# SnappyDataInc/snappydata

Hardware: AMD Instinct MI355X
Metric: rows/sec scan+filter+agg (TPC-H lineitem) (higher is better)
Workload: dtype f64; 1 GPU; tpch_q6_lineitem_sf100; rows_per_gpu=600000000, total_rows=600000000, bytes_per_row=28, batch_rows=600000, parallelism=bucket-dp1, jit=True

## Files before the change

### include/snappy_engine.h

```cpp
#ifndef SNAPPY_ENGINE_H
#define SNAPPY_ENGINE_H

#include <stdint.h>
#include <stddef.h>

#ifdef __cplusplus
extern "C" {
#endif

#define SN_OK                0
#define SN_ERR_GENERIC      -1
#define SN_ERR_BADARG       -2
#define SN_ERR_NOMEM        -3
#define SN_ERR_BADFORMAT    -4
#define SN_ERR_UNSUPPORTED  -5
#define SN_ERR_NOGPU        -6
#define SN_ERR_OVERFLOW     -7

typedef enum {
  SN_TYPE_INT32  = 0,
  SN_TYPE_INT64  = 1,
  SN_TYPE_DOUBLE = 2,
  SN_TYPE_STRING = 3,
  SN_TYPE_BOOL   = 4,
// ... 135 lines not shown
                           double *dict, int32_t *ndict);

int32_t sn_dim_define(sn_engine *e, const char *name);
int32_t sn_dim_put(sn_engine *e, int32_t dim, int64_t nkeys,
                   const int64_t *keys, const char *attr_payload,
                   const int32_t *attr_lens);

int32_t sn_dim_from_table(sn_engine *e, int32_t dim, int32_t table,
                          int32_t key_col, int32_t attr_col);

int32_t sn_batch_mutate(sn_engine *e, int32_t table, int64_t uuid,
                        int32_t bucket_id, const sn_buf *delete_mask,
                        const sn_buf *deltas, const sn_buf *stats);

sn_query *sn_query_submit(sn_engine *e, const sn_plan *plan);
int32_t   sn_query_wait(sn_query *q);
int32_t   sn_query_result(sn_query *q, sn_result *out);
void      sn_query_destroy(sn_query *q);
double    sn_query_kernel_ms(sn_query *q);
int32_t   sn_query_result_page(sn_query *q, int64_t offset, sn_result *out);
int64_t   sn_query_num_groups(sn_query *q);
int32_t   sn_query_used_jit(sn_query *q);
int64_t   sn_query_late_cols(sn_query *q);
int32_t   sn_query_order_by(sn_query *q, int32_t agg_idx, int32_t descending,
                            int64_t k);

int64_t sn_query_partial_bytes(sn_query *q);
int32_t sn_query_partials(sn_query *q, void *dst, int32_t dst_is_device);
int64_t sn_query_partial_bytes2(sn_query *q, int32_t cap_slots);
int32_t sn_query_partials2(sn_query *q, void *dst, int32_t dst_is_device,
                           int32_t cap_slots);
int32_t sn_query_partials_sharded2(sn_query *q, int32_t world, void *dst,
                                   int32_t cap_slots);
int32_t sn_query_partials_sharded(sn_query *q, int32_t world, void *dst);
int32_t sn_query_merge(sn_query *q, const void *blocks, int64_t stride,
                       int32_t n_blocks);

typedef struct {
  int32_t col, _pad;
  int64_t add, mul;
} sn_dec_factor;

typedef struct {
  int32_t kind, nfactors;
  sn_dec_factor factors[SN_MAX_FACTORS];
} sn_dec_agg;
// ... 57 lines not shown
```

### snappydata_amd/csrc/engine.cpp

```cpp
#include <hip/hip_runtime.h>
#include <dlfcn.h>

#include <algorithm>
#include <atomic>
#include <climits>
#include <cmath>
#include <cstdarg>
#include <cstdio>
#include <cstring>
#include <malloc.h>
#include <limits>
#include <map>
#include <set>
#include <memory>
#include <mutex>
#include <string>
#include <thread>
#include <vector>

#include "../../include/snappy_engine.h"
#include "engine_internal.h"
#include "blob_format.h"
#include "partial_format.h"

// ... 148 lines not shown
  std::vector<int64_t> keys;
  std::vector<std::string> attrs;
  std::vector<std::string> attr_dict;
  std::vector<int32_t> attr_gid;
  const int64_t *dev_keys = nullptr;
  const int32_t *dev_payload = nullptr;
  int32_t cap_log2 = 0;
  const int32_t *dev_lut = nullptr;
  int64_t lut_min = 0, lut_max = -1;
  int32_t attr_maxlen = 0;
  bool from_table = false;
  std::mutex mu;
};

struct sn_engine {
  sn_config cfg;
  Arena arena;
  std::vector<std::unique_ptr<Table>> tables;
  std::vector<std::unique_ptr<Dim>> dims;
  hipStream_t stream = nullptr;
  bool has_gpu = false;
  bool narrow = true;
  bool late = true, late_force = false;
  double *scratch = nullptr;
  size_t scratch_sz = 0;
  long long *hws_keys = nullptr;
  long long *hws_okeys = nullptr;
  double *hws_acc = nullptr;
  double *hws_orows = nullptr;
  int32_t *hws_flags = nullptr;
  int hws_cap_log2 = 0;
  size_t hws_acc_bytes = 0;
  double *rws_recs = nullptr;
  size_t rws_bytes = 0;
  int32_t *rws_pcount = nullptr;
  int rws_npart = 0;
  int32_t *lz4_err_dev = nullptr;
  std::mutex lz4_mu;
  std::mutex query_mu;
  static const int PIN_SLOTS = 4;
  struct PinSlot { void *buf = nullptr; size_t sz = 0; std::mutex mu; };
  PinSlot pins[PIN_SLOTS];
  std::atomic<uint32_t> pin_rr { 0 };
  void *jit = nullptr;
  std::map<uint64_t, void *> dp_cache;
  std::vector<hipEvent_t> ev_pool;
// ... 10 lines not shown
  }
  void ev_release(hipEvent_t ev) {
    if (!ev) return;
    std::lock_guard<std::mutex> g(aux_mu);
    if (ev_pool.size() < 16) ev_pool.push_back(ev);
    else (void)hipEventDestroy(ev);
  }
};

extern "C" sn_engine *sn_engine_create(const sn_config *cfg) {
  auto *e = new sn_engine();
  if (cfg) e->cfg = *cfg;
  else memset(&e->cfg, 0, sizeof(e->cfg));
  if (e->cfg.column_batch_size <= 0) e->cfg.column_batch_size = 24ll << 20;
  if (e->cfg.column_max_delta_rows <= 0) e->cfg.column_max_delta_rows = 10000;
  if (e->cfg.hash_join_size <= 0) e->cfg.hash_join_size = 100ll << 20;
  if (e->cfg.shard_count <= 0) e->cfg.shard_count = 1;
  if (e->cfg.n_buckets <= 0) e->cfg.n_buckets = 128;
  if (const char *nv = getenv("SN_NARROW")) e->narrow = nv[0] != '0';
  if (const char *lv = getenv("SN_LATE")) {
    e->late = lv[0] != '0';
    e->late_force = !strcmp(lv, "force");
  }
  int ndev = 0;
  if (hipGetDeviceCount(&ndev) == hipSuccess && ndev > 0 && e->cfg.device >= 0) {
    if (hipSetDevice(e->cfg.device) == hipSuccess &&
        hipStreamCreate(&e->stream) == hipSuccess) {
      e->has_gpu = true;
      e->arena.device = e->cfg.device;
    }
  }
  if (!e->has_gpu) {
    e->arena.device = -1;
  } else {
    e->jit = sn_jit_cache_create();
  }
  (void)mallopt(M_MMAP_THRESHOLD, 256 << 20);
  (void)mallopt(M_TRIM_THRESHOLD, 256 << 20);
  return e;
}

static hipError_t d2h_copy(sn_engine *e, void *dst, const void *src, size_t n) {
  if (n < (1u << 20))
    return hipMemcpy(dst, src, n, hipMemcpyDeviceToHost);
  auto &slot = e->pins[e->pin_rr.fetch_add(1) % sn_engine::PIN_SLOTS];
  std::lock_guard<std::mutex> g(slot.mu);
// ... 1173 lines not shown
  bool mm = false;
  std::unique_ptr<long long[]> sparse_keys;
  std::unique_ptr<double[]> sparse_rows;
  size_t sparse_n = 0;
  std::vector<double> sparse_null_row;
  bool gint[2] = { false, false };
  int64_t gmin[2] = { 0, 0 };
  int gnull1 = -1, gnull2 = -1;
  int agg_map[SN_MAX_AGGS];
  int dev_naggs = 0;
  Dim *join_dim = nullptr;
  bool join_group = false;
  double *dev_out = nullptr;
  size_t out_stride = 0;
  int na_t = 0;
  std::vector<double> host_out;
  int64_t rows_scanned = 0;
  int64_t batches_seen = 0, batches_skipped = 0;
  hipEvent_t ev_start = nullptr, ev_stop = nullptr;
  std::vector<std::pair<void *, size_t>> owned;
  float kernel_ms = -1.0f;
  bool used_jit = false;
  int64_t late_cols = 0;
  bool done = false;
  bool merged = false;
  std::vector<GroupOut> final_groups;
  bool dec = false;
  int dec_ndev = 0;
  int dec_map[SN_MAX_AGGS];
  int dec_scale_of[SN_MAX_AGGS];
  unsigned long long *dec_out = nullptr;
  std::vector<sn_dec_val> dec_vals;
  bool select = false;
  int sel_nproj = 0;
  int32_t sel_cols[SN_SEL_MAX_PROJ];
  int64_t sel_limit = 0;
  int64_t sel_total = 0;
  int64_t sel_rows = 0;
  int sel_width[SN_SEL_MAX_PROJ];
  void *sel_val[SN_SEL_MAX_PROJ];
  uint8_t *sel_valid[SN_SEL_MAX_PROJ];
  int sel_kernels = 0;
  bool ordered = false;
  int32_t ord_col = 0, ord_flags = 0;
  int32_t rjoin = -1;
  float sel_ms[3] = { 0.0f, 0.0f, 0.0f };
// ... 927 lines not shown
}

static uint32_t tag_late_columns(const sn_query *q, const sn_dev_plan &dp,
                                 int *kinds) {
  const sn_engine *e = q->e;
  const sn_plan *plan = &q->plan;
  if (!e->late || plan->ngroup > 0 || q->join_dim || q->sparse || dp.nslots > 1)
    return 0;
  uint32_t agg = 0, other = 0;
  for (int a = 0; a < dp.naggs; a++) {
    const sn_dev_agg &A = dp.aggs[a];
    if (A.nf >= 1) agg |= 1u << A.c0;
    if (A.nf >= 2) agg |= 1u << A.c1;
    if (A.nf >= 3) agg |= 1u << A.c2;
  }
  for (int i = 0; i < dp.npreds_d; i++) other |= 1u << dp.preds_d[i].cslot;
  for (int i = 0; i < dp.npreds_i; i++) other |= 1u << dp.preds_i[i].cslot;
  for (int i = 0; i < dp.npreds_in && i < 2; i++) other |= 1u << dp.inp[i].cslot;
  uint32_t mask = 0;
  for (int ui = 0; ui < dp.nused; ui++)
    if (kinds[ui] == SN_K_F64 && ((agg & ~other) >> ui & 1)) mask |= 1u << ui;
  if (!mask || !other) return 0;
  if (!e->late_force && !(estimate_selectivity(q) <= SN_LATE_MAX_SEL)) return 0;
  for (int ui = 0; ui < dp.nused; ui++)
    if ((mask >> ui) & 1) kinds[ui] = SN_K_F64_LATE;
  return mask;
}

static int32_t launch_dense(sn_query *q, const sn_dev_plan &dp,
                            const ScanSet &set) {
  sn_engine *e = q->e;
  const int32_t ntiles = set.ntiles;
  size_t out_n = (size_t)q->nslots * q->out_stride;
  q->dev_out = (double *)e->arena.alloc(out_n * 8);
  if (!q->dev_out) return fail(SN_ERR_NOMEM, "out alloc");
  q->owned.push_back({ q->dev_out, out_n * 8 });
  if (hipMemsetAsync(q->dev_out, 0, out_n * 8, e->stream) != hipSuccess)
    return fail(SN_ERR_GENERIC, "memset out");
  if (ntiles == 0) return SN_OK;
  void *dp_dev = cached_dev_plan(e, dp);
  if (!dp_dev) return fail(SN_ERR_NOMEM, "plan upload");
  const sn_dense_launch d = sn_dense_launch_of(&dp, ntiles);
  const size_t rows = (size_t)std::max(sn_dense_rows(&d, 0), sn_dense_rows(&d, 1));
  int rc = ensure_scratch(e, rows * d.nv * 8);
  if (rc != SN_OK) return rc;
  if (d.global_acc &&
      hipMemsetAsync(e->scratch, 0, rows * d.nv * 8, e->stream) != hipSuccess)
    return fail(SN_ERR_GENERIC, "accumulator zero");
  if (d.global_acc && q->mm &&
      sn_launch_acc_init(e->scratch, (long long)rows * dp.nslots, q->dev_naggs,
                         d.na1, dp_dev, e->stream) != 0)
    return fail(SN_ERR_GENERIC, "accumulator min/max init");
  acquire_events(q);
  void *jfn = nullptr;
  uint32_t late = 0;
  if (e->jit && sn_jit_shape_ok(&dp) && jit_inlists_ok(dp) && set.jit_ok) {
    int kinds[SN_DEV_MAX_COLS];
    memcpy(kinds, set.jit_kinds, sizeof(kinds));
    late = tag_late_columns(q, dp, kinds);
    jfn = sn_jit_get(e->jit, &dp, kinds, dp.nslots, q->na_t, set.jit_del);
  }
  if (jfn)
    for (size_t ui = 0; ui < q->used_cols.size(); ui++)
      if (((late >> ui) & 1) && q->used_cols[ui] < 63)
        q->late_cols |= 1ll << q->used_cols[ui];
  if (q->ev_start) (void)hipEventRecord(q->ev_start, e->stream);
  rc = -1;
  if (jfn) {
    rc = sn_jit_launch(jfn, d.grid_compiled, (const sn_dev_batch *)set.db_dev,
                       (const sn_dev_tile *)set.tl_dev, ntiles, e->scratch,
                       dp.jkeys, dp.jpayload, dp.jlut,
                       (const sn_dev_plan *)dp_dev, e->stream);
    if (rc == 0)
      rc = sn_launch_reduce(e->scratch, sn_dense_rows(&d, 1), d.nv,
                            q->dev_out, d.naggs1, d.out_stride,
                            dp_dev, e->stream);
    q->used_jit = rc == 0;
    if (rc != 0) jfn = nullptr;
  }
  if (!jfn)
    rc = sn_launch_scan_agg(&dp, (const sn_dev_plan *)dp_dev,
                            (const sn_dev_batch *)set.db_dev,
                            (const sn_dev_tile *)set.tl_dev, ntiles,
                            q->dev_out, e->scratch, e->stream);
  if (q->ev_stop) (void)hipEventRecord(q->ev_stop, e->stream);
  if (rc != 0)
    return fail(SN_ERR_GENERIC, "kernel launch: %s", hipGetErrorString((hipError_t)rc));
  return SN_OK;
}

static sn_query *submit_impl(sn_engine *e, const sn_plan *plan,
                             const DecReq *dec) {
  if (!e || !plan) { fail(SN_ERR_BADARG, "null engine/plan"); return nullptr; }
  Table *t = get_table(e, plan->table);
  if (!t) { fail(SN_ERR_BADARG, "unknown table %d", plan->table); return nullptr; }
  if (!e->has_gpu) { fail(SN_ERR_NOGPU, "no HIP device — the engine never falls back to CPU"); return nullptr; }
  std::lock_guard<std::mutex> qg(e->query_mu);
  if (plan->npreds > SN_MAX_PREDS || plan->naggs > SN_MAX_AGGS ||
      plan->ngroup > SN_MAX_GROUPS || plan->naggs <= 0) {
    fail(SN_ERR_BADARG, "plan limits exceeded"); return nullptr;
// ... 890 lines not shown
  int32_t rc = q->select ? wait_select(q)
               : q->dec  ? wait_decimal(q) : wait_f64(q);
  if (rc != SN_OK) return rc;
  if (q->ev_start && q->ev_stop)
    (void)hipEventElapsedTime(&q->kernel_ms, q->ev_start, q->ev_stop);
  q->done = true;
  return SN_OK;
}

extern "C" double sn_query_kernel_ms(sn_query *q) {
  if (!q) return -1.0;
  (void)sn_query_wait(q);
  return (double)q->kernel_ms;
}

extern "C" int32_t sn_query_used_jit(sn_query *q) {
  return q && q->used_jit ? 1 : 0;
}

extern "C" int64_t sn_query_late_cols(sn_query *q) {
  return q && q->used_jit ? q->late_cols : 0;
}

extern "C" int32_t sn_engine_jit_count(sn_engine *e) {
  return e ? sn_jit_cache_count(e->jit) : 0;
}

static int eff_ngroup(const sn_query *q) {
  return q->join_group ? 1 + q->plan.ngroup : q->plan.ngroup;
}

static AccRowLayout row_layout(const sn_query *q) {
  const sn_plan &p = q->plan;
  AccRowLayout L;
  L.form = q->sparse ? SN_ROW_SPARSE
           : eff_ngroup(q) == 0 ? SN_ROW_KEYLESS : SN_ROW_DENSE;
  L.naggs = p.naggs; L.na_t = q->na_t; L.dev_naggs = q->dev_naggs;
  L.pac = q->pac;
  for (int a = 0; a < SN_MAX_AGGS; a++) {
    L.agg_map[a] = q->agg_map[a];
    L.kinds[a] = p.aggs[a].kind;
  }
  L.rowcount_at = acc_rowcount_at(L.form, L.na_t, L.dev_naggs, L.pac);
  return L;
}

// ... 285 lines not shown
```

### snappydata_amd/csrc/engine_internal.h

```cpp
#ifndef SN_ENGINE_INTERNAL_H
#define SN_ENGINE_INTERNAL_H

#include <stdint.h>
#include <stdlib.h>

#include "../../include/snappy_engine.h"

static inline int sn_type_width(sn_type_t dtype) {
  switch (dtype) {
    case SN_TYPE_DOUBLE: case SN_TYPE_INT64: return 8;
    case SN_TYPE_INT32: case SN_TYPE_FLOAT: return 4;
    case SN_TYPE_INT16: return 2;
    case SN_TYPE_INT8: case SN_TYPE_BOOL: return 1;
    default: return 0;
  }
}

#define SN_LUT_MAX_SPAN (1ll << 24)
static inline int64_t sn_lut_span(int64_t mn, int64_t mx) {
  if (mx < mn) return 0;
  const uint64_t d = (uint64_t)mx - (uint64_t)mn;
  return d < (uint64_t)SN_LUT_MAX_SPAN ? (int64_t)d + 1 : 0;
}

#define SN_DEV_MAX_COLS 8

enum {
  SN_K_F64 = 0, SN_K_I32 = 1, SN_K_I64 = 2, SN_K_F32 = 3,
  SN_K_DICT16 = 4,
  SN_K_DICT32 = 5,
  SN_K_I16 = 6, SN_K_BOOLBIT = 7,
  SN_K_U8 = 8,
  SN_K_S8 = 9,
  SN_K_RLE = 10,
  SN_K_RLE_I64 = 11,
  SN_K_F64C8 = 12,
  SN_K_F64_LATE = 13
};

typedef struct {
  const void     *body;
  const uint64_t *nullw;
  const uint32_t *nullpfx;
  const int32_t  *dictmap;
  const uint64_t *patch_bm;
  const int32_t  *patch_pos;
  const double   *patch_val;
  const uint64_t *patch_nullbm;
  const int32_t *rle_ends;
  const double  *rle_vals;
  int32_t rle_n;
  int32_t patch_n;
  int32_t kind;
  int32_t has_nulls;
  int32_t null_gid;
} sn_dev_col;

typedef struct {
  int32_t num_rows;
  int32_t clean;
// ... 465 lines not shown
                             long long dlen, int32_t *err, void *stream);

int sn_launch_col_minmax(const void *body, long long n, int kind,
                         unsigned long long *omin, unsigned long long *omax,
                         void *stream);

#define SN_NARROW_MAX 256
int sn_launch_f64_narrow(const double *body, long long n, unsigned char *codes,
                         double *dict, int *ndict, void *stream);

int sn_launch_reduce(const double *dev_scratch, int nblocks, int nv,
                     double *dev_out, int naggs1, int out_stride,
                     const void *plan_dev, void *stream);

int sn_launch_acc_init(double *acc, long long rows, int naggs, int na1,
                       const void *plan_dev, void *stream);

int sn_jit_shape_ok(const sn_dev_plan *p);
void *sn_jit_cache_create(void);
void sn_jit_cache_destroy(void *cache);
int sn_jit_cache_count(void *cache);
void *sn_jit_get(void *cache, const sn_dev_plan *p, const int *kinds,
                 int nslots, int na_t, int has_del);
int sn_jit_launch(void *fn, int grid, const sn_dev_batch *batches,
                  const sn_dev_tile *tiles, int ntiles, double *scratch,
                  const int64_t *jkeys, const int32_t *jpayload,
                  const int32_t *jlut, const sn_dev_plan *plan_dev,
                  void *stream);

#ifdef __cplusplus
}
#endif
#endif
```

### snappydata_amd/csrc/jit.cpp

```cpp
#include <hip/hip_runtime.h>
#include <hip/hiprtc.h>

#include <cstdarg>
#include <cstddef>
#include <cstdio>
#include <cstring>
#include <cstdlib>
#include <map>
#include <mutex>
#include <string>
#include <vector>

#include "engine_internal.h"

struct JitFn {
  hipModule_t mod = nullptr;
  hipFunction_t fn = nullptr;
};

struct JitCache {
  std::map<uint64_t, JitFn> fns;
  std::mutex mu;
};

extern "C" void *sn_jit_cache_create(void) { return new JitCache(); }
extern "C" void sn_jit_cache_destroy(void *c) {
  auto *jc = (JitCache *)c;
  if (!jc) return;
  for (auto &kv : jc->fns)
    if (kv.second.mod) (void)hipModuleUnload(kv.second.mod);
  delete jc;
}

__attribute__((format(printf, 1, 2)))
static std::string strf(const char *fmt, ...) {
  va_list ap, ap2;
  va_start(ap, fmt);
  va_copy(ap2, ap);
  const int n = vsnprintf(nullptr, 0, fmt, ap);
  va_end(ap);
  std::string s(n > 0 ? (size_t)n + 1 : 0, '\0');
  if (n > 0) vsnprintf(&s[0], s.size(), fmt, ap2), s.resize((size_t)n);
  va_end(ap2);
  return s;
}
#define emitf(o, ...) ((o) += strf(__VA_ARGS__))


#define JIT_CHUNK 1024
#define JIT_WG 256
#define JIT_MAX_AGGS 12
#define JIT_REG_MAX_SLOTS 8
#define JIT_REG_MAX_AGGS 6
#define JIT_LDS_MAX_SLOTS 1024
#define JIT_LDS_BUDGET (160 * 1024)
#define JIT_SLUT_MAX_BYTES (100 * 1024)

enum JitAcc {
  ACC_KEYLESS,
  ACC_REGS,
  ACC_WBIN,
  ACC_LDS,
  ACC_GLOBAL,
  ACC_SPARSE,
  ACC_RADIX
};

enum JitProbe {
  PROBE_NONE,
  PROBE_HASH,
  PROBE_SPAY,
  PROBE_SLUT
};

enum JitSlot {
  SLOT_NONE,
  SLOT_SINGLE,
  SLOT_DENSE,
  SLOT_JOIN_ATTR,
  SLOT_SPARSE_PROBE,
  SLOT_RADIX_RANK
};

struct JitShape {
  int NC, NA;
  int NS, NA1;
  int nv;
  int mm_any;
  JitAcc acc;
  JitProbe probe;
  JitSlot slot;
  long long slut_span, slut_words;
  int occupancy;
  int nlate;
  int nstaged;
  int lds_dict;
  int late[SN_DEV_MAX_COLS];
  int srow[SN_DEV_MAX_COLS];
};

static JitAcc jit_acc_mode(int nslots, int naggs, int pac, int sparse,
                           int radix, int mm_any) {
  if (sparse) return radix ? ACC_RADIX : ACC_SPARSE;
  if (nslots <= 1 && !pac) return ACC_KEYLESS;
  if (nslots > JIT_LDS_MAX_SLOTS) return ACC_GLOBAL;
  if (nslots > JIT_REG_MAX_SLOTS) return ACC_LDS;
  if (naggs <= 2 && !mm_any && nslots * (naggs + 1) >= 12) return ACC_WBIN;
  return ACC_REGS;
}

extern "C" int sn_jit_shape_ok(const sn_dev_plan *p) {
  const int naggs = p->naggs, nslots = p->nslots;
  const int na1 = p->pac ? 2 * naggs + 1 : naggs + 1;
  switch (jit_acc_mode(nslots, naggs, p->pac != 0, p->sparse != 0, 0, 0)) {
    case ACC_KEYLESS: case ACC_SPARSE: case ACC_RADIX:
      return naggs <= JIT_MAX_AGGS;
    case ACC_REGS: case ACC_WBIN: return naggs <= JIT_REG_MAX_AGGS;
    case ACC_LDS:
      return (size_t)p->nused * JIT_CHUNK * 8 + (size_t)nslots * na1 * 8 + 1024
// ... 32 lines not shown
            : slut ? PROBE_SLUT : p->jlut ? PROBE_SPAY : PROBE_HASH;

  if (sparse) s.slot = s.acc == ACC_RADIX ? SLOT_RADIX_RANK : SLOT_SPARSE_PROBE;
  else if (s.acc == ACC_KEYLESS) s.slot = SLOT_NONE;
  else if (p->jkeys && p->jmode == 1) s.slot = SLOT_JOIN_ATTR;
  else s.slot = p->ngroup == 0 ? SLOT_SINGLE : SLOT_DENSE;

  static const int spocc_env = [] {
    const char *v = getenv("SN_JIT_SPOCC");
    return v ? atoi(v) : 0;
  }();
  if (sparse) s.occupancy = spocc_env > 0 ? spocc_env : 4;
  else if (s.acc == ACC_LDS || s.acc == ACC_GLOBAL) s.occupancy = 1;
  else s.occupancy = s.acc == ACC_WBIN ? 4 : 2;

  const bool late_mode = s.probe == PROBE_NONE &&
      (s.acc == ACC_KEYLESS || (s.acc == ACC_REGS && s.slot == SLOT_SINGLE));
  unsigned pred_cols = 0;
  for (int i = 0; i < p->npreds_d; i++) pred_cols |= 1u << p->preds_d[i].cslot;
  for (int i = 0; i < p->npreds_i; i++) pred_cols |= 1u << p->preds_i[i].cslot;
  for (int i = 0; i < p->npreds_in && i < 2; i++)
    pred_cols |= 1u << p->inp[i].cslot;
  s.nlate = 0;
  for (int c = 0; c < s.NC; c++)
    s.nlate += s.late[c] = late_mode && kinds[c] == SN_K_F64_LATE &&
                           !((pred_cols >> c) & 1);
  if (s.nlate == s.NC) {
    s.nlate = 0;
    for (int c = 0; c < s.NC; c++) s.late[c] = 0;
  }
  s.nstaged = 0;
  for (int c = 0; c < s.NC; c++) s.srow[c] = s.late[c] ? -1 : s.nstaged++;
  static const int lds_dict_env = [] {
    const char *v = getenv("SN_JIT_LATE_LDSDICT");
    return !v || v[0] != '0';
  }();
  s.lds_dict = s.nlate > 0 && lds_dict_env;
  return s;
}

enum JitConv {
  CV_BITS64,
  CV_NUM,
  CV_F32,
  CV_DICT,
  CV_VDICT
};
struct JitKind {
  const char *reg;
  int bytes;
  const char *mem;
  JitConv conv;
  int i64;
  int store_each;
};
static const JitKind &jit_kind(int k) {
  static const JitKind f64 = { "double2_t", 8, "double", CV_BITS64, 0, 0 };
  static const JitKind i64 = { "double2_t", 8, "double", CV_BITS64, 1, 0 };
  static const JitKind i32 = { "int2_t", 4, "int", CV_NUM, 0, 1 };
  static const JitKind f32 = { "int2_t", 4, "float", CV_F32, 0, 0 };
  static const JitKind d32 = { "int2_t", 4, "int", CV_DICT, 0, 0 };
  static const JitKind d16 = { "unsigned", 2, "unsigned short", CV_DICT, 0, 0 };
  static const JitKind i16 = { "unsigned", 2, "short", CV_NUM, 0, 0 };
  static const JitKind c8 = { "unsigned short", 1, "unsigned char", CV_VDICT,
                              0, 0 };
  switch (k) {
    case SN_K_F64: case SN_K_F64_LATE: return f64;
    case SN_K_I64: return i64;
    case SN_K_I32: return i32;
    case SN_K_F32: return f32;
    case SN_K_DICT32: return d32;
    case SN_K_DICT16: return d16;
    case SN_K_F64C8: return c8;
    default: return i16;
  }
}

static std::string kind_reg_row(const JitKind &K, int c, int j) {
  if (K.bytes == 2)
    return strf((j & 1) ? "st%d_%d >> 16" : "st%d_%d & 0xffff", c, j >> 1);
  if (K.bytes == 1)
    return strf((j & 1) ? "st%d_%d >> 8" : "st%d_%d & 0xff", c, j >> 1);
  return strf("st%d_%d.%s", c, j >> 1, (j & 1) ? "y" : "x");
}

static std::string kind_image_from_reg(const JitKind &K, int c, int j) {
  const std::string r = kind_reg_row(K, c, j);
  switch (K.conv) {
    case CV_BITS64: return r;
    case CV_DICT: return strf("(double)dm%d[%s]", c, r.c_str());
// ... 440 lines not shown
}

static void emit_spay_from_image(Gen &g) {
  emitf(g.o, "      if (!staged) {\n"
           "#pragma unroll\n"
           "        for (int k = 0; k < CHUNK / WG; k++) {\n"
           "          const int r = tid + k * WG;\n"
           "          const double jx = sval[%d][r];\n",
        g.p->jcslot);
  emit_lut_probe(g, plan_col_is_i64(g.p, g.p->jcslot)
                        ? "__double_as_longlong(jx)" : "(i64)jx",
                 "spay[r]", "          ");
  g.o += "        }\n"
         "      }\n";
}

static void emit_radix_stash(Gen &g) {
  emitf(g.o, "      i64 rkey[CHUNK / WG];\n"
           "      int rok[CHUNK / WG], rpk[CHUNK / WG], rrnk[CHUNK / WG];\n");
  for (int a = 0; a < g.s.NA; a++)
    emitf(g.o, "      double rva%d[CHUNK / WG];\n", a);
}

static void emit_row_predicates(Gen &g) {
  std::string &o = g.o;
  const sn_dev_plan *p = g.p;
  if (g.has_del)
    o += "        if (del) {\n"
         "          const int gr = base + r;\n"
         "          ok &= (int)(~(del[(u64)gr >> 6] >> (gr & 63)) & 1ull);\n"
         "        }\n";
  for (int i = 0; i < p->npreds_d; i++) {
    emitf(o, "        { const double x = sval[%d][r];\n"
             "          ok &= (x >= pd%d_lo) & (x <= pd%d_hi); }\n",
          g.s.srow[p->preds_d[i].cslot], i, i);
  }
  for (int i = 0; i < p->npreds_i; i++) {
    emitf(o, "        { const i64 x = __double_as_longlong(sval[%d][r]);\n"
             "          ok &= (x >= pi%d_lo) & (x <= pi%d_hi); }\n",
          g.s.srow[p->preds_i[i].cslot], i, i);
  }
  for (int i = 0; i < p->npreds_in && i < 2; i++) {
    const int cs = p->inp[i].cslot;
    const int is64 = plan_col_is_i64(p, cs);
    emitf(o, "        { const i64 v = %ssval[%d][r]%s;\n"
             "          const i64 ix = v - inb%d_base;\n"
             "          ok &= (ix >= 0) & (ix < inb%d_lim) &\n"
             "                (int)((inbm%d[ix >> 6] >> (ix & 63)) & 1ull); }\n",
          is64 ? "__double_as_longlong(" : "(i64)", g.s.srow[cs],
          is64 ? ")" : "", i, i, i);
  }
}

static void emit_late_stash(Gen &g) {
// ... 120 lines not shown
)";
      break;
    case SLOT_JOIN_ATTR:
      if (p->jslot_mul > 0 && p->ngroup >= 1)
        emitf(o, "        const int slot = (pay > 0 ? pay : 0) * %d +"
                 " (int)((i64)sval[%d][r] - %lldll);\n",
              p->jslot_mul, p->gcol[0], (long long)p->gbase[0]);
      else
        o += "        const int slot = pay > 0 ? pay : 0;\n";
      break;
    case SLOT_SINGLE:
      o += "        const int slot = 0;\n";
      break;
    case SLOT_DENSE:
      emitf(o, "        int slot = (int)(((i64)sval[%d][r] - %lldll) * %d);\n",
            p->gcol[0], (long long)p->gbase[0], p->gmul0 ? p->gmul0 : 1);
      if (p->ngroup >= 2)
        emitf(o, "        slot += (int)((i64)sval[%d][r] - %lldll);\n",
              p->gcol[1], (long long)p->gbase[1]);
      break;
  }
}

static void emit_agg_values(Gen &g) {
  std::string &o = g.o;
  auto factor = [&](int a, int i, int cs, double fa, double fm) {
    const std::string f = g.s.late[cs] ? strf("e%d[k]", cs)
        : plan_col_is_i64(g.p, cs)
        ? strf("(double)__double_as_longlong(sval[%d][r])", g.s.srow[cs])
        : strf("sval[%d][r]", g.s.srow[cs]);
    if (ftriv(fa, fm)) return f;
    return strf("__builtin_fma(ag%d_m%d, %s, ag%d_a%d)", a, i, f.c_str(), a, i);
  };
  for (int a = 0; a < g.s.NA; a++) {
    const sn_dev_agg &A = g.p->aggs[a];
    if (A.nf < 1) { emitf(o, "        const double va%d = 1.0;\n", a); continue; }
    emitf(o, "        %sdouble va%d = %s", g.s.acc == ACC_REGS ? "" : "const ", a,
          factor(a, 0, A.c0, A.a0, A.m0).c_str());
    if (A.nf >= 2) emitf(o, " * %s", factor(a, 1, A.c1, A.a1, A.m1).c_str());
    if (A.nf >= 3) emitf(o, " * %s", factor(a, 2, A.c2, A.a2, A.m2).c_str());
    o += ";\n";
  }
}

static void emit_accumulate(Gen &g) {
  std::string &o = g.o;
  const JitShape &s = g.s;
  switch (s.acc) {
    case ACC_RADIX:
      for (int a = 0; a < s.NA; a++)
// ... 135 lines not shown
        for (int a = 0; a < s.NA; a++)
          emitf(o, "        atomicAdd(&bacc[s * %d + %d], x);\n", s.NA1, s.NA + a);
      o += "      } }\n  }\n";
      emit_store_row(g, "bacc[i]");
      break;
    case ACC_KEYLESS:
      emit_acc_init(o, g, "bacc", s.nv, 0);
      for (int a = 0; a < s.NA; a++) {
        emitf(o, "  { double x = wsum(sums[%d]);\n"
                 "    if ((tid & 63) == 0 && x != 0.0) atomicAdd(&bacc[%d], x); }\n", a, a);
        emitf(o, "  { double x = wsum(cnts[%d]);\n"
                 "    if ((tid & 63) == 0 && x != 0.0) atomicAdd(&bacc[%d], x); }\n",
              a, g.na_t + a);
      }
      emitf(o, "  { double x = wsum(rcnt);\n"
               "    if ((tid & 63) == 0 && x != 0.0) atomicAdd(&bacc[%d], x); }\n",
            2 * g.na_t);
      emit_store_row(g, "bacc[i]");
      break;
  }
  o += "}\n";
}

static std::string gen_source(const sn_dev_plan *p, const int *kinds,
                              int nslots, int na_t, int has_del) {
  Gen g = { std::string(), p, kinds, na_t, has_del,
            jit_classify(p, kinds, nslots, na_t, has_del) };
  std::string &o = g.o;
  const bool radix = g.s.acc == ACC_RADIX;

  emit_prelude(o);
  for (int c = 0; c < g.s.NC; c++)
    if (jit_kind(kinds[c]).conv == CV_VDICT) {
      emitf(o, "static_assert(__builtin_offsetof(sn_dev_col, rle_vals) == %zu, "
               "\"layout mirror differs from engine_internal.h\");\n",
            offsetof(sn_dev_col, rle_vals));
      break;
    }
  emit_order_helpers(g);
  emit_signature(g);
  emit_literals(g);
  emit_acc_decl(g);
  emit_probe_decl(g);
  emit_stage_regs(g);
  if (g.s.probe == PROBE_SLUT) emit_slut_pack(g);

  emit_tile_prologue(g);
  o += "    int staged = 0;\n"
       "    if (tile.row_start + CHUNK <= tile_end) {\n";
  emit_stage_load(g, "tile.row_start", "      ");
  o += "      staged = 1;\n    }\n"
       "    for (int base = tile.row_start; base < tile_end; base += CHUNK) {\n"
       "      const int rows = min(CHUNK, tile_end - base);\n";
  if (radix)
    o += "      for (int i = tid; i < npart; i += WG) phist[i] = 0;\n";
  o += "      if (staged) {\n";
  if (g.s.probe == PROBE_SPAY) emit_spay_from_regs(g);
  emit_stage_write(g, "        ");
  o += "      } else {\n";
  emit_scalar_tail(g);
  o += "      }\n"
// ... 99 lines not shown
  hiprtcResult crc = hiprtcCompileProgram(prog, 2, opts);
  if (crc != HIPRTC_SUCCESS) {
    size_t lsz = 0;
    hiprtcGetProgramLogSize(prog, &lsz);
    std::vector<char> log(lsz + 1, 0);
    if (lsz) hiprtcGetProgramLog(prog, log.data());
    fprintf(stderr, "[sn_jit] compile failed:\n%s\n", log.data());
    hiprtcDestroyProgram(&prog);
    jc->fns[h] = JitFn();
    return nullptr;
  }
  size_t csz = 0;
  hiprtcGetCodeSize(prog, &csz);
  std::vector<char> code(csz);
  hiprtcGetCode(prog, code.data());
  hiprtcDestroyProgram(&prog);

  JitFn jf;
  if (hipModuleLoadData(&jf.mod, code.data()) != hipSuccess) return nullptr;
  if (hipModuleGetFunction(&jf.fn, jf.mod, "jit_scan") != hipSuccess) {
    (void)hipModuleUnload(jf.mod);
    return nullptr;
  }
  jc->fns[h] = jf;
  return (void *)jf.fn;
}

extern "C" int sn_jit_cache_count(void *cache) {
  auto *jc = (JitCache *)cache;
  if (!jc) return 0;
  std::lock_guard<std::mutex> g(jc->mu);
  return (int)jc->fns.size();
}

extern "C" int sn_jit_launch(void *fn, int grid,
                             const sn_dev_batch *batches,
                             const sn_dev_tile *tiles, int ntiles,
                             double *scratch, const int64_t *jkeys,
                             const int32_t *jpayload, const int32_t *jlut,
                             const sn_dev_plan *plan_dev, void *stream) {
  void *args[] = { (void *)&batches, (void *)&tiles, (void *)&ntiles,
                   (void *)&scratch, (void *)&jkeys, (void *)&jpayload,
                   (void *)&jlut, (void *)&plan_dev };
  hipError_t e = hipModuleLaunchKernel((hipFunction_t)fn, grid, 1, 1,
                                       256, 1, 1, 0, (hipStream_t)stream,
                                       args, nullptr);
  return (int)e;
}
// ... 1 lines not shown
```

### snappydata_amd/engine.py

```python
import ctypes as C
import os
import subprocess

import numpy as np

from . import abi

_DIR = os.path.dirname(os.path.abspath(__file__))
_SO = os.path.join(_DIR, "libsnappy_engine.so")


class EngineError(RuntimeError):
    def __init__(self, code, msg=""):
        super().__init__(f"engine error {code}: {msg}")
        self.code = code


def build(force=False):
    srcdir = os.path.join(_DIR, "csrc")
    srcs = [os.path.join(srcdir, f) for f in
            ("engine.cpp", "builder.cpp", "jit.cpp", "kernels.hip",
             "engine_internal.h", "blob_format.h", "partial_format.h")]
    srcs.append(os.path.join(os.path.dirname(_DIR), "include",
                             "snappy_engine.h"))
# ... 31 lines not shown
        L.sn_table_num_rows.argtypes = [C.c_void_p, C.c_int32]
        L.sn_table_narrowed_batches.restype = C.c_int64
        L.sn_table_narrowed_batches.argtypes = [C.c_void_p, C.c_int32,
                                                C.c_int32]
        L.sn_f64_narrow_host.restype = None
        L.sn_f64_narrow_host.argtypes = [C.c_void_p, C.c_int64, C.c_void_p,
                                         C.c_void_p, C.c_void_p]
        L.sn_table_get_blob.restype = C.c_int64
        L.sn_table_get_blob.argtypes = [C.c_void_p, C.c_int32, C.c_int32,
                                        C.c_int32, C.c_void_p, C.c_int64]
        L.sn_query_submit.restype = C.c_void_p
        L.sn_query_submit.argtypes = [C.c_void_p, C.POINTER(abi.SnPlan)]
        L.sn_query_wait.restype = C.c_int32
        L.sn_query_wait.argtypes = [C.c_void_p]
        L.sn_query_result.restype = C.c_int32
        L.sn_query_result.argtypes = [C.c_void_p, C.POINTER(abi.SnResult)]
        L.sn_query_destroy.argtypes = [C.c_void_p]
        L.sn_query_kernel_ms.restype = C.c_double
        L.sn_query_kernel_ms.argtypes = [C.c_void_p]
        L.sn_query_used_jit.restype = C.c_int32
        L.sn_query_used_jit.argtypes = [C.c_void_p]
        L.sn_query_late_cols.restype = C.c_int64
        L.sn_query_late_cols.argtypes = [C.c_void_p]
        L.sn_query_order_by.restype = C.c_int32
        L.sn_query_order_by.argtypes = [C.c_void_p, C.c_int32, C.c_int32,
                                        C.c_int64]
        L.sn_query_result_page.restype = C.c_int32
        L.sn_query_result_page.argtypes = [C.c_void_p, C.c_int64,
                                           C.POINTER(abi.SnResult)]
        L.sn_query_num_groups.restype = C.c_int64
        L.sn_query_num_groups.argtypes = [C.c_void_p]
        L.sn_engine_jit_count.restype = C.c_int32
        L.sn_engine_jit_count.argtypes = [C.c_void_p]
        L.sn_query_partial_bytes.restype = C.c_int64
        L.sn_query_partial_bytes.argtypes = [C.c_void_p]
        L.sn_query_partials.restype = C.c_int32
        L.sn_query_partials.argtypes = [C.c_void_p, C.c_void_p, C.c_int32]
        L.sn_query_merge.restype = C.c_int32
        L.sn_query_merge.argtypes = [C.c_void_p, C.c_void_p, C.c_int64, C.c_int32]
        L.sn_query_partials_sharded.restype = C.c_int32
        L.sn_query_partials_sharded.argtypes = [C.c_void_p, C.c_int32, C.c_void_p]
        L.sn_query_partial_bytes2.restype = C.c_int64
        L.sn_query_partial_bytes2.argtypes = [C.c_void_p, C.c_int32]
        L.sn_query_partials2.restype = C.c_int32
        L.sn_query_partials2.argtypes = [C.c_void_p, C.c_void_p, C.c_int32,
                                         C.c_int32]
# ... 223 lines not shown
        naggs = len(self.dec_aggs)
        out = []
        v = abi.SnDecVal()
        for r, (keys, _vals) in enumerate(keyrows):
            ints, scales = [], []
            for a in range(naggs):
                _check(lib().sn_query_result_dec(self._h, r, a, C.byref(v)),
                       "query_result_dec")
                ints.append(abi.dec_int(v))
                scales.append(int(v.scale))
            out.append((keys, ints, scales))
        return out

    def kernel_ms(self):
        return lib().sn_query_kernel_ms(self._h)

    def used_jit(self):
        return bool(lib().sn_query_used_jit(self._h))

    def late_cols(self):
        m = int(lib().sn_query_late_cols(self._h))
        return [c for c in range(63) if (m >> c) & 1]

    def order_by(self, agg_idx, descending=False, k=0):
        _check(lib().sn_query_order_by(self._h, agg_idx,
                                       1 if descending else 0, k), "order_by")
        return self

    def num_groups(self):
        return _check(lib().sn_query_num_groups(self._h), "num_groups")

    def partial_bytes(self, cap=None):
        if cap is None:
            return _check(lib().sn_query_partial_bytes(self._h))
        return _check(lib().sn_query_partial_bytes2(self._h, cap))

    def partials_host(self, cap=None):
        n = self.partial_bytes(cap)
        buf = np.zeros(n, dtype=np.uint8)
        if cap is None:
            _check(lib().sn_query_partials(self._h, buf.ctypes.data, 0),
                   "partials")
        else:
            _check(lib().sn_query_partials2(self._h, buf.ctypes.data, 0, cap),
                   "partials")
        return buf
# ... 317 lines not shown
```

Measured before the change: 518.5 billion rows/s.

## Add direct register-staged JIT kernel path with prefetch and residency-sized grid

Adds a new JIT code generator for keyless late-materialized scans. It loads narrow predicate columns straight into registers in DS-row slices and prefetches the next slice. Dictionary predicates become LDS ballot bitmasks, and f64 aggregate columns are fetched only for passing rows. It also sizes the launch grid to the occupancy-derived resident block count. The aim is to cut the LDS staging and sync overhead and the tail imbalance of the generic kernel, at the cost of more register pressure and another code path to maintain.

```diff
diff --git a/include/snappy_engine.h b/include/snappy_engine.h
--- a/include/snappy_engine.h
+++ b/include/snappy_engine.h
@@ -181,6 +181,7 @@
 int64_t   sn_query_num_groups(sn_query *q);
 int32_t   sn_query_used_jit(sn_query *q);
 int64_t   sn_query_late_cols(sn_query *q);
+int32_t   sn_query_direct(sn_query *q);
 int32_t   sn_query_order_by(sn_query *q, int32_t agg_idx, int32_t descending,
                             int64_t k);
 
diff --git a/snappydata_amd/csrc/engine.cpp b/snappydata_amd/csrc/engine.cpp
--- a/snappydata_amd/csrc/engine.cpp
+++ b/snappydata_amd/csrc/engine.cpp
@@ -194,6 +194,7 @@
   bool has_gpu = false;
   bool narrow = true;
   bool late = true, late_force = false;
+  bool direct = true, grid_resident = true;
   double *scratch = nullptr;
   size_t scratch_sz = 0;
   long long *hws_keys = nullptr;
@@ -250,6 +251,8 @@
     e->late = lv[0] != '0';
     e->late_force = !strcmp(lv, "force");
   }
+  if (const char *dv = getenv("SN_DIRECT")) e->direct = dv[0] != '0';
+  if (const char *gv = getenv("SN_GRID_RESIDENT")) e->grid_resident = gv[0] != '0';
   int ndev = 0;
   if (hipGetDeviceCount(&ndev) == hipSuccess && ndev > 0 && e->cfg.device >= 0) {
     if (hipSetDevice(e->cfg.device) == hipSuccess &&
@@ -1469,6 +1472,7 @@
   float kernel_ms = -1.0f;
   bool used_jit = false;
   int64_t late_cols = 0;
+  int direct = 0;
   bool done = false;
   bool merged = false;
   std::vector<GroupOut> final_groups;
@@ -2442,8 +2446,14 @@
     if (kinds[ui] == SN_K_F64 && ((agg & ~other) >> ui & 1)) mask |= 1u << ui;
   if (!mask || !other) return 0;
   if (!e->late_force && !(estimate_selectivity(q) <= SN_LATE_MAX_SEL)) return 0;
+  bool direct = e->direct && !q->mm && !dp.pac && dp.npreds_i == 0 &&
+                dp.npreds_in == 0;
+  for (int ui = 0; ui < dp.nused && direct; ui++)
+    direct = ((mask >> ui) & 1) || kinds[ui] == SN_K_I32 ||
+             kinds[ui] == SN_K_I16 || kinds[ui] == SN_K_F64C8;
   for (int ui = 0; ui < dp.nused; ui++)
-    if ((mask >> ui) & 1) kinds[ui] = SN_K_F64_LATE;
+    if ((mask >> ui) & 1)
+      kinds[ui] = direct ? SN_K_F64_LATE_DIRECT : SN_K_F64_LATE;
   return mask;
 }
 
@@ -2460,7 +2470,23 @@
   if (ntiles == 0) return SN_OK;
   void *dp_dev = cached_dev_plan(e, dp);
   if (!dp_dev) return fail(SN_ERR_NOMEM, "plan upload");
-  const sn_dense_launch d = sn_dense_launch_of(&dp, ntiles);
+  sn_dense_launch d = sn_dense_launch_of(&dp, ntiles);
+  void *jfn = nullptr;
+  uint32_t late = 0;
+  bool direct = false;
+  if (e->jit && sn_jit_shape_ok(&dp) && jit_inlists_ok(dp) && set.jit_ok) {
+    int kinds[SN_DEV_MAX_COLS];
+    memcpy(kinds, set.jit_kinds, sizeof(kinds));
+    late = tag_late_columns(q, dp, kinds);
+    for (int ui = 0; ui < dp.nused; ui++)
+      direct |= kinds[ui] == SN_K_F64_LATE_DIRECT;
+    jfn = sn_jit_get(e->jit, &dp, kinds, dp.nslots, q->na_t, set.jit_del);
+  }
+  if (jfn && e->grid_resident && d.route == SN_ROUTE_KEYLESS) {
+    const int resident = sn_jit_resident(e->jit, jfn);
+    if (resident > 0 && resident <= SN_GRID_CAP)
+      d.grid_compiled = sn_balanced_grid(ntiles, resident);
+  }
   const size_t rows = (size_t)std::max(sn_dense_rows(&d, 0), sn_dense_rows(&d, 1));
   int rc = ensure_scratch(e, rows * d.nv * 8);
   if (rc != SN_OK) return rc;
@@ -2472,14 +2498,6 @@
                          d.na1, dp_dev, e->stream) != 0)
     return fail(SN_ERR_GENERIC, "accumulator min/max init");
   acquire_events(q);
-  void *jfn = nullptr;
-  uint32_t late = 0;
-  if (e->jit && sn_jit_shape_ok(&dp) && jit_inlists_ok(dp) && set.jit_ok) {
-    int kinds[SN_DEV_MAX_COLS];
-    memcpy(kinds, set.jit_kinds, sizeof(kinds));
-    late = tag_late_columns(q, dp, kinds);
-    jfn = sn_jit_get(e->jit, &dp, kinds, dp.nslots, q->na_t, set.jit_del);
-  }
   if (jfn)
     for (size_t ui = 0; ui < q->used_cols.size(); ui++)
       if (((late >> ui) & 1) && q->used_cols[ui] < 63)
@@ -2496,6 +2514,7 @@
                             q->dev_out, d.naggs1, d.out_stride,
                             dp_dev, e->stream);
     q->used_jit = rc == 0;
+    q->direct = rc == 0 && direct;
     if (rc != 0) jfn = nullptr;
   }
   if (!jfn)
@@ -3432,6 +3451,10 @@
   return q && q->used_jit ? q->late_cols : 0;
 }
 
+extern "C" int32_t sn_query_direct(sn_query *q) {
+  return q && q->used_jit ? q->direct : 0;
+}
+
 extern "C" int32_t sn_engine_jit_count(sn_engine *e) {
   return e ? sn_jit_cache_count(e->jit) : 0;
 }
diff --git a/snappydata_amd/csrc/engine_internal.h b/snappydata_amd/csrc/engine_internal.h
--- a/snappydata_amd/csrc/engine_internal.h
+++ b/snappydata_amd/csrc/engine_internal.h
@@ -35,7 +35,8 @@
   SN_K_RLE = 10,
   SN_K_RLE_I64 = 11,
   SN_K_F64C8 = 12,
-  SN_K_F64_LATE = 13
+  SN_K_F64_LATE = 13,
+  SN_K_F64_LATE_DIRECT = 14
 };
 
 typedef struct {
@@ -547,6 +548,7 @@
 int sn_jit_cache_count(void *cache);
 void *sn_jit_get(void *cache, const sn_dev_plan *p, const int *kinds,
                  int nslots, int na_t, int has_del);
+int sn_jit_resident(void *cache, void *fn);
 int sn_jit_launch(void *fn, int grid, const sn_dev_batch *batches,
                   const sn_dev_tile *tiles, int ntiles, double *scratch,
                   const int64_t *jkeys, const int32_t *jpayload,
diff --git a/snappydata_amd/csrc/jit.cpp b/snappydata_amd/csrc/jit.cpp
--- a/snappydata_amd/csrc/jit.cpp
+++ b/snappydata_amd/csrc/jit.cpp
@@ -16,6 +16,7 @@
 struct JitFn {
   hipModule_t mod = nullptr;
   hipFunction_t fn = nullptr;
+  int resident = 0;
 };
 
 struct JitCache {
@@ -49,6 +50,7 @@
 
 #define JIT_CHUNK 1024
 #define JIT_WG 256
+#define JIT_DIRECT_SLOTS 8
 #define JIT_MAX_AGGS 12
 #define JIT_REG_MAX_SLOTS 8
 #define JIT_REG_MAX_AGGS 6
@@ -95,6 +97,7 @@
   int nlate;
   int nstaged;
   int lds_dict;
+  int direct;
   int late[SN_DEV_MAX_COLS];
   int srow[SN_DEV_MAX_COLS];
 };
@@ -173,9 +176,12 @@
   for (int i = 0; i < p->npreds_in && i < 2; i++)
     pred_cols |= 1u << p->inp[i].cslot;
   s.nlate = 0;
-  for (int c = 0; c < s.NC; c++)
-    s.nlate += s.late[c] = late_mode && kinds[c] == SN_K_F64_LATE &&
-                           !((pred_cols >> c) & 1);
+  int direct_tag = 0;
+  for (int c = 0; c < s.NC; c++) {
+    direct_tag |= kinds[c] == SN_K_F64_LATE_DIRECT;
+    s.nlate += s.late[c] = late_mode && !((pred_cols >> c) & 1) &&
+        (kinds[c] == SN_K_F64_LATE || kinds[c] == SN_K_F64_LATE_DIRECT);
+  }
   if (s.nlate == s.NC) {
     s.nlate = 0;
     for (int c = 0; c < s.NC; c++) s.late[c] = 0;
@@ -187,6 +193,8 @@
     return !v || v[0] != '0';
   }();
   s.lds_dict = s.nlate > 0 && lds_dict_env;
+  s.direct = direct_tag && s.nlate > 0 && s.acc == ACC_KEYLESS;
+  if (s.direct) s.lds_dict = 0;
   return s;
 }
 
@@ -216,7 +224,7 @@
   static const JitKind c8 = { "unsigned short", 1, "unsigned char", CV_VDICT,
                               0, 0 };
   switch (k) {
-    case SN_K_F64: case SN_K_F64_LATE: return f64;
+    case SN_K_F64: case SN_K_F64_LATE: case SN_K_F64_LATE_DIRECT: return f64;
     case SN_K_I64: return i64;
     case SN_K_I32: return i32;
     case SN_K_F32: return f32;
@@ -703,14 +711,18 @@
     emitf(g.o, "      double rva%d[CHUNK / WG];\n", a);
 }
 
+static void emit_delete_pred(Gen &g) {
+  if (g.has_del)
+    g.o += "        if (del) {\n"
+           "          const int gr = base + r;\n"
+           "          ok &= (int)(~(del[(u64)gr >> 6] >> (gr & 63)) & 1ull);\n"
+           "        }\n";
+}
+
 static void emit_row_predicates(Gen &g) {
   std::string &o = g.o;
   const sn_dev_plan *p = g.p;
-  if (g.has_del)
-    o += "        if (del) {\n"
-         "          const int gr = base + r;\n"
-         "          ok &= (int)(~(del[(u64)gr >> 6] >> (gr & 63)) & 1ull);\n"
-         "        }\n";
+  emit_delete_pred(g);
   for (int i = 0; i < p->npreds_d; i++) {
     emitf(o, "        { const double x = sval[%d][r];\n"
              "          ok &= (x >= pd%d_lo) & (x <= pd%d_hi); }\n",
@@ -877,10 +889,136 @@
   }
 }
 
+
+static bool direct_has_pred(const Gen &g, int c) {
+  for (int i = 0; i < g.p->npreds_d; i++)
+    if (g.p->preds_d[i].cslot == c) return true;
+  return false;
+}
+
+static bool direct_is_factor(const Gen &g, int c) {
+  for (int a = 0; a < g.s.NA; a++) {
+    const sn_dev_agg &A = g.p->aggs[a];
+    if ((A.nf >= 1 && A.c0 == c) || (A.nf >= 2 && A.c1 == c) ||
+        (A.nf >= 3 && A.c2 == c))
+      return true;
+  }
+  return false;
+}
+
+static std::string direct_factor(const Gen &g, int cs) {
+  return jit_kind(g.kinds[cs]).conv == CV_VDICT
+             ? strf("svd%d[pb][f%d[k]]", cs, cs)
+             : strf("(double)f%d[k]", cs);
+}
+
+static const char *direct_reg_type(const JitKind &K) {
+  return K.conv == CV_VDICT ? "unsigned" : "int";
+}
+
+static void emit_direct_decl(Gen &g) {
+  std::string &o = g.o;
+  const JitShape &s = g.s;
+  static_assert(JIT_WG == SN_NARROW_MAX, "one dictionary entry per lane");
+  for (int c = 0; c < s.NC; c++) {
+    if (jit_kind(g.kinds[c]).conv != CV_VDICT) continue;
+    if (direct_is_factor(g, c))
+      emitf(o, "  __shared__ __attribute__((aligned(16))) double svd%d[2][WG];\n", c);
+    if (direct_has_pred(g, c))
+      emitf(o, "  __shared__ __attribute__((aligned(16))) u64 spass%d[2][4];\n", c);
+  }
+  emitf(o, "  __shared__ __attribute__((aligned(16))) double bacc[%d];\n", s.nv);
+  o += "  const int tid = threadIdx.x;\n";
+  emitf(o, "  double sums[%d], cnts[%d], rcnt = 0.0;\n", s.NA, s.NA);
+  emitf(o, "#pragma unroll\n  for (int a = 0; a < %d; a++) { sums[a] = 0; cnts[a] = 0; }\n", s.NA);
+  o += "  int pb = 0;\n";
+  for (int c = 0; c < s.NC; c++)
+    if (!s.late[c])
+      emitf(o, "  %s x%d[DS];\n", direct_reg_type(jit_kind(g.kinds[c])), c);
+}
+
+static void emit_direct_dicts(Gen &g) {
+  std::string &o = g.o;
+  const sn_dev_plan *p = g.p;
+  for (int c = 0; c < g.s.NC; c++) {
+    if (jit_kind(g.kinds[c]).conv != CV_VDICT) continue;
+    if (direct_is_factor(g, c))
+      emitf(o, "    svd%d[pb][tid] = vd%d[tid];\n", c, c);
+    if (!direct_has_pred(g, c)) continue;
+    emitf(o, "    { const double x = vd%d[tid];\n"
+             "      int in = 1;\n", c);
+    for (int i = 0; i < p->npreds_d; i++)
+      if (p->preds_d[i].cslot == c)
+        emitf(o, "      in &= (x >= pd%d_lo) & (x <= pd%d_hi);\n", i, i);
+    emitf(o, "      const u64 m = __ballot(in);\n"
+             "      if ((tid & 63) == 0) spass%d[pb][tid >> 6] = m; }\n", c);
+  }
+  o += "    __syncthreads();\n";
+  for (int c = 0; c < g.s.NC; c++)
+    if (jit_kind(g.kinds[c]).conv == CV_VDICT && direct_has_pred(g, c))
+      emitf(o, "    const unsigned *pw%d = (const unsigned *)spass%d[pb];\n", c, c);
+}
+
+static void emit_direct_load(Gen &g, const char *base_expr, const char *ind) {
+  std::string &o = g.o;
+  emitf(o, "%sif (%s < tile_end) {\n"
+           "#pragma unroll\n"
+           "%s  for (int k = 0; k < DS; k++) {\n"
+           "%s    const unsigned rr = min((unsigned)(tid + k * WG),\n"
+           "%s                            (unsigned)(tile_end - 1 - (%s)));\n",
+        ind, base_expr, ind, ind, ind, base_expr);
+  for (int c = 0; c < g.s.NC; c++) {
+    if (g.s.late[c]) continue;
+    const JitKind &K = jit_kind(g.kinds[c]);
+    emitf(o, "%s    x%d[k] = ((const GAS %s *)(body%d + (u64)(%s) * %d))[rr];\n",
+          ind, c, K.mem, c, base_expr, K.bytes);
+  }
+  emitf(o, "%s  }\n%s}\n", ind, ind);
+}
+
+static void emit_direct_pass_a(Gen &g) {
+  std::string &o = g.o;
+  const sn_dev_plan *p = g.p;
+  o += "      int okv[DS];\n";
+  for (int c = 0; c < g.s.NC; c++) {
+    if (g.s.late[c]) emitf(o, "      double e%d[DS];\n", c);
+    else if (direct_is_factor(g, c))
+      emitf(o, "      %s f%d[DS];\n", direct_reg_type(jit_kind(g.kinds[c])), c);
+  }
+  o += "#pragma unroll\n"
+       "      for (int k = 0; k < DS; k++) {\n"
+       "        const int r = tid + k * WG;\n"
+       "        int ok = base + r < tile_end;\n";
+  emit_delete_pred(g);
+  for (int c = 0; c < g.s.NC; c++) {
+    if (g.s.late[c] || !direct_has_pred(g, c)) continue;
+    if (jit_kind(g.kinds[c]).conv == CV_VDICT) {
+      emitf(o, "        ok &= (int)((pw%d[x%d[k] >> 5] >> (x%d[k] & 31u)) & 1u);\n",
+            c, c, c);
+      continue;
+    }
+    for (int i = 0; i < p->npreds_d; i++)
+      if (p->preds_d[i].cslot == c)
+        emitf(o, "        { const double x = (double)x%d[k];\n"
+                 "          ok &= (x >= pd%d_lo) & (x <= pd%d_hi); }\n", c, i, i);
+  }
+  o += "        okv[k] = ok;\n";
+  for (int c = 0; c < g.s.NC; c++) {
+    if (g.s.late[c])
+      emitf(o, "        e%d[k] = 0.0;\n"
+               "        if (ok) e%d[k] = ((const GAS double *)(body%d + (u64)base * 8))[r];\n",
+            c, c, c);
+    else if (direct_is_factor(g, c))
+      emitf(o, "        f%d[k] = x%d[k];\n", c, c);
+  }
+  o += "      }\n";
+}
+
 static void emit_agg_values(Gen &g) {
   std::string &o = g.o;
   auto factor = [&](int a, int i, int cs, double fa, double fm) {
     const std::string f = g.s.late[cs] ? strf("e%d[k]", cs)
+        : g.s.direct ? direct_factor(g, cs)
         : plan_col_is_i64(g.p, cs)
         ? strf("(double)__double_as_longlong(sval[%d][r])", g.s.srow[cs])
         : strf("sval[%d][r]", g.s.srow[cs]);
@@ -1062,6 +1200,50 @@
   o += "}\n";
 }
 
+static int direct_slots(void) {
+  static const int v = [] {
+    const char *e = getenv("SN_DIRECT_SLOTS");
+    const int n = e ? atoi(e) : 0;
+    return n == 4 || n == 8 || n == 16 ? n : JIT_DIRECT_SLOTS;
+  }();
+  return v;
+}
+static int direct_prefetch(void) {
+  static const int v = [] {
+    const char *e = getenv("SN_DIRECT_PREFETCH");
+    return !e || e[0] != '0';
+  }();
+  return v;
+}
+
+static void gen_direct(Gen &g) {
+  std::string &o = g.o;
+  g.s.occupancy = 32 / direct_slots();
+  emitf(o, "#define DS %d\n", direct_slots());
+  emit_signature(g);
+  emit_literals(g);
+  emit_direct_decl(g);
+  emit_tile_prologue(g);
+  emit_direct_dicts(g);
+  emit_direct_load(g, "tile.row_start", "    ");
+  o += "    for (int base = tile.row_start; base < tile_end; base += DS * WG) {\n";
+  emit_direct_pass_a(g);
+  o += "      const int nbase = base + DS * WG;\n";
+  if (direct_prefetch()) emit_direct_load(g, "nbase", "      ");
+  o += "#pragma unroll\n"
+       "      for (int k = 0; k < DS; k++) {\n"
+       "        const int ok = okv[k];\n"
+       "        if (__popcll(__ballot(ok)) == 0) continue;\n";
+  emit_agg_values(g);
+  emit_accumulate(g);
+  o += "      }\n";
+  if (!direct_prefetch()) emit_direct_load(g, "nbase", "      ");
+  o += "    }\n"
+       "    pb ^= 1;\n"
+       "  }\n";
+  emit_flush(g);
+}
+
 static std::string gen_source(const sn_dev_plan *p, const int *kinds,
                               int nslots, int na_t, int has_del) {
   Gen g = { std::string(), p, kinds, na_t, has_del,
@@ -1077,6 +1259,10 @@
             offsetof(sn_dev_col, rle_vals));
       break;
     }
+  if (g.s.direct) {
+    gen_direct(g);
+    return std::move(g.o);
+  }
   emit_order_helpers(g);
   emit_signature(g);
   emit_literals(g);
@@ -1222,8 +1408,24 @@
     (void)hipModuleUnload(jf.mod);
     return nullptr;
   }
+  int per_cu = 0, dev = 0, cus = 0;
+  if (hipModuleOccupancyMaxActiveBlocksPerMultiprocessor(&per_cu, jf.fn, JIT_WG,
+                                                         0) == hipSuccess &&
+      per_cu > 0 && hipGetDevice(&dev) == hipSuccess &&
+      hipDeviceGetAttribute(&cus, hipDeviceAttributeMultiprocessorCount,
+                            dev) == hipSuccess && cus > 0)
+    jf.resident = per_cu * cus;
   jc->fns[h] = jf;
   return (void *)jf.fn;
+}
+
+extern "C" int sn_jit_resident(void *cache, void *fn) {
+  auto *jc = (JitCache *)cache;
+  if (!jc || !fn) return 0;
+  std::lock_guard<std::mutex> g(jc->mu);
+  for (const auto &kv : jc->fns)
+    if ((void *)kv.second.fn == fn) return kv.second.resident;
+  return 0;
 }
 
 extern "C" int sn_jit_cache_count(void *cache) {
diff --git a/snappydata_amd/engine.py b/snappydata_amd/engine.py
--- a/snappydata_amd/engine.py
+++ b/snappydata_amd/engine.py
@@ -77,6 +77,8 @@
         L.sn_query_used_jit.argtypes = [C.c_void_p]
         L.sn_query_late_cols.restype = C.c_int64
         L.sn_query_late_cols.argtypes = [C.c_void_p]
+        L.sn_query_direct.restype = C.c_int32
+        L.sn_query_direct.argtypes = [C.c_void_p]
         L.sn_query_order_by.restype = C.c_int32
         L.sn_query_order_by.argtypes = [C.c_void_p, C.c_int32, C.c_int32,
                                         C.c_int64]
@@ -346,6 +348,9 @@
         m = int(lib().sn_query_late_cols(self._h))
         return [c for c in range(63) if (m >> c) & 1]
 
+    def direct(self):
+        return int(lib().sn_query_direct(self._h))
+
     def order_by(self, agg_idx, descending=False, k=0):
         _check(lib().sn_query_order_by(self._h, agg_idx,
                                        1 if descending else 0, k), "order_by")
```

Result: faster. 644.3 billion rows/s, median of 6 (+24.3%).
